# Qiyuan-Ge/PaintMind

Measured on AMD Instinct MI355X. Metric: 256x256 images/sec, 8-step MaskGIT decode (vit-s-vqgan), whole job, higher is better.
Workload: dtype bf16; 1 GPU; maskgit-uncond-12L-d512-T8; batch_per_gpu=64, topk=5, decode=every step (reference-equivalent work), parallelism=dp1 (independent images, no data-path collective), hip_graph=True, concurrent_micro_batches=2, dispatch_mode=AMD_DIRECT_DISPATCH=1 (default), rank_mode=False

## Files before the change

paintmind_amd/csrc/gemm.hip:

```cpp
#include <stdlib.h>

#include "gemm_common.h"

using namespace pmgemm;

int pm_gemm256_supported(const GemmParams& p, int dtype, int epi, int out_dtype);
int pm_gemm256_launch(const GemmParams& p, int epi, int out_dtype, hipStream_t s);
int pm_gemm2b_supported(const GemmParams& p, int dtype, int epi, int out_dtype);
int pm_gemm2b_launch(const GemmParams& p, int epi, int out_dtype, hipStream_t s);

namespace {

constexpr int BM = 128, BN = 128;
constexpr int TILE_BYTES = 128 * ROWB;
constexpr int STAGE_BYTES = 2 * TILE_BYTES;
constexpr int THREADS = 256;

template <typename T, int CH = 4>
__device__ __forceinline__ void stage_tile(const T* __restrict__ base, int ld, int row0, int rows_total,
                                           int k0, unsigned char* lds_tile, int wave, int lane) {
#pragma unroll
    for (int i = 0; i < CH; ++i) {
        const int chunk = wave * CH + i;
        const int r = chunk * 8 + (lane >> 3);
        const int slot = (lane & 7) ^ (r & 7);
        int gr = row0 + r;
        gr = gr < rows_total ? gr : rows_total - 1;
        const unsigned char* src =
            reinterpret_cast<const unsigned char*>(base + (size_t)gr * ld + k0) + slot * 16;
        glds16(src, lds_tile + chunk * 1024);
    }
}

template <typename T, int EPI, typename OutT, bool FOLD = false, int STAGES = 2, int WM = 2>
__global__ __launch_bounds__(WM * 128) void gemm_nt_kernel(const GemmParams p) {
    static_assert(STAGES == 2 || (STAGES == 4 && sizeof(T) == 2), "the four-stage K loop is the bf16 small-batch form");
    static_assert(WM == 2 || (WM == 4 && STAGES == 4), "eight waves only in the latency form");
    constexpr int MI = 8 / WM;
    constexpr int CH = 8 / WM;
    __shared__ __attribute__((aligned(1024))) unsigned char lds[STAGES * STAGE_BYTES];

    const int tid = threadIdx.x;
    const int lane = tid & 63;
    const int wave = __builtin_amdgcn_readfirstlane(tid >> 6);
    const int wm = wave >> 1, wn = wave & 1;
    const int l15 = lane & 15, g = lane >> 4;

    const int tiles_n = (p.N + BN - 1) / BN, tiles_m = (p.M + BM - 1) / BM;
    int tm, tn;
    tile_of_block(xcd_remap(blockIdx.x, gridDim.x), tiles_m, tiles_n, 8, tm, tn);
    const int m0 = tm * BM, n0 = tn * BN;

    const T* A = reinterpret_cast<const T*>(p.A);
    const T* W = reinterpret_cast<const T*>(p.W);
    constexpr int KSTEP = ROWB / (int)sizeof(T);
    const int nk = p.K / KSTEP;

    f32x4_t acc[MI][4];
#pragma unroll
    for (int i = 0; i < MI; ++i)
#pragma unroll
        for (int j = 0; j < 4; ++j) acc[i][j] = f32x4_t{0.f, 0.f, 0.f, 0.f};

    constexpr bool RPRE = (EPI == EPI_STD && sizeof(OutT) == 4);
    float4 rpre[RPRE ? MI * 4 : 1];
    if constexpr (RPRE) {
        if (p.residual) {
            const int ncol = n0 + wn * 64 + (lane & 15) * 4;
#pragma unroll
            for (int mi = 0; mi < MI; ++mi)
#pragma unroll
                for (int it = 0; it < 4; ++it) {
                    int mm = m0 + wm * (MI * 16) + mi * 16 + it * 4 + (lane >> 4);
                    mm = mm < p.M ? mm : p.M - 1;
                    const int nc = ncol < p.N ? ncol : 0;
                    rpre[mi * 4 + it] = *reinterpret_cast<const float4*>(p.residual + (size_t)(mm % p.res_rows) * p.ldr + nc);
                }
        }
    }

    stage_tile<T, CH>(A, p.lda, m0, p.M, 0, lds, wave, lane);
    stage_tile<T, CH>(W, p.ldw, n0, p.N, 0, lds + TILE_BYTES, wave, lane);

    [[maybe_unused]] float4 fcc[FOLD ? 4 : 1], fdd[FOLD ? 4 : 1];
    [[maybe_unused]] float2 fab[FOLD ? MI : 1];
    [[maybe_unused]] float2 fpa[FOLD && STAGES == 4 ? MI : 1][8], fpb[FOLD && STAGES == 4 ? MI : 1][8];
    if constexpr (FOLD) {
#pragma unroll
        for (int ni = 0; ni < 4; ++ni) {
            fcc[ni] = *reinterpret_cast<const float4*>(p.ln_c + n0 + wn * 64 + ni * 16 + g * 4);
// ... 114 lines not shown
        if (p.out_lo) { wave_epilogue<EPI, OutT, MI, 1, false, 2, NoHook, STAGES != 4>(p, acc, eraw, m0 + wm * (MI * 16), n0 + wn * 64, lane, rpre); return; }
    }
    wave_epilogue<EPI, OutT, MI, RPRE ? MI * 4 : 1, false, -1, NoHook, STAGES != 4>(p, acc, eraw, m0 + wm * (MI * 16), n0 + wn * 64, lane, rpre);
}

int tiles128(const GemmParams& p) { return ceil_div(p.M, BM) * ceil_div(p.N, BN); }


bool deep128(const GemmParams& p) {
    static const int deep_max = pm_dev_knob("PMHIP_GEMM128_DEEP_MAX_TILES", 256);
    return tiles128(p) <= deep_max && p.K >= 4 * 64;
}

template <typename T, int EPI, typename OutT, bool FOLD = false>
int launch(const GemmParams& p, bool deep, hipStream_t s) {
    const int tiles = tiles128(p);
    PmTimer tm(gemm_family(p, EPI), s);
    if constexpr (sizeof(T) == 2) {
        if (deep) {
            hipLaunchKernelGGL((gemm_nt_kernel<T, EPI, OutT, FOLD, 4, 4>), dim3(tiles), dim3(512), 0, s, p);
            PM_HIP(hipGetLastError());
            return PMHIP_OK;
        }
    }
    hipLaunchKernelGGL((gemm_nt_kernel<T, EPI, OutT, FOLD>), dim3(tiles), dim3(THREADS), 0, s, p);
    PM_HIP(hipGetLastError());
    return PMHIP_OK;
}

bool fold_small(const GemmParams& p) {
    static const int max_tiles = pm_dev_knob("PMHIP_FOLD128_MAX_TILES", 128);
    return (p.M / 256) * (p.N / 256) <= max_tiles;
}

bool use256(const GemmParams& p, int dtype, int epi, int out_dtype) {
    static const int g_use256 = pm_dev_knob("PMHIP_GEMM256", 1);
    return g_use256 && pm_gemm256_supported(p, dtype, epi, out_dtype);
}

bool use2b(const GemmParams& p, int dtype, int epi, int out_dtype) {
    static const int g_use2b = pm_dev_knob("PMHIP_GEMM2B", 1);
    if (!g_use2b || !pm_gemm2b_supported(p, dtype, epi, out_dtype)) return false;
    if (g_use2b >= 2) return true;
    return epi == EPI_STD && p.residual && !pm_gemm256_supported(p, dtype, epi, out_dtype);
}

int check_common(const GemmParams& p, int dtype) {
    PM_REQUIRE(dtype == PMHIP_F32 || dtype == PMHIP_BF16, "gemm: bad dtype %d", dtype);
    PM_REQUIRE(p.M > 0 && p.N > 0 && p.K > 0, "gemm: empty problem M=%d N=%d K=%d", p.M, p.N, p.K);
    PM_REQUIRE(p.K % 64 == 0, "gemm: K=%d must be a multiple of 64 (pad on the host)", p.K);
    PM_REQUIRE(p.lda % 8 == 0 && p.ldw % 8 == 0, "gemm: lda/ldw must be multiples of 8 elements");
    PM_REQUIRE(p.lda >= p.K, "gemm: lda=%d is smaller than K=%d (rows of A would overlap)", p.lda, p.K);
    PM_REQUIRE(p.ldw >= p.K, "gemm: ldw=%d is smaller than K=%d (rows of W would overlap)", p.ldw, p.K);
    PM_REQUIRE(p.A && p.W, "gemm: null operand");
    return PMHIP_OK;
}

int set_lnfold(GemmParams& p, const pmhip_lnfold* ln, int dtype) {
    PM_REQUIRE(ln->coef && ln->c && ln->d, "gemm_ln: null fold pointer");
    PM_REQUIRE(dtype == PMHIP_BF16, "gemm_ln: the LayerNorm fold exists in bf16 mode only");
    PM_REQUIRE(p.K % 128 == 0, "gemm_ln: K=%d must be a multiple of 128", p.K);
    p.ln_c = ln->c; p.ln_d = ln->d; p.ln_coef = ln->coef;
    PM_REQUIRE(pm_lnfold_shape_ok(p.M, p.N, p.K, p.lda, p.ldw),
               "gemm_ln: shape M=%d N=%d K=%d is not served by the 256x256 kernel (M, N multiples of 256)", p.M, p.N, p.K);
    PM_REQUIRE(!ln->parts || (ln->nparts > 0 && ln->nparts <= 16 && ln->nparts * 64 == p.K), "gemm_ln: nparts=%d does not describe K=%d columns",
               ln->nparts, p.K);
    return PMHIP_OK;
}

template <int EPI, bool FOLD>
int launch_bf16(const GemmParams& p, int out_dtype, bool deep, hipStream_t s) {
    if constexpr (EPI == EPI_STD)
        if (out_dtype == PMHIP_F32) return launch<bf16_t, EPI, float, FOLD>(p, deep, s);
    return launch<bf16_t, EPI, bf16_t, FOLD>(p, deep, s);
}

template <int EPI>
int dispatch(GemmParams& p, int dtype, int out_dtype, const pmhip_lnfold* ln, pmhip_stream stream) {
    hipStream_t s = (hipStream_t)stream;
    if (ln) {
        PM_TRY(set_lnfold(p, ln, dtype));
        const bool small = fold_small(p), deep = small && deep128(p);
        if (ln->parts) {
            if (deep) { p.ln_parts = ln->parts; p.ln_nparts = ln->nparts; p.ln_eps = ln->eps; p.ln_coef_out = const_cast<float*>(ln->coef); }
            else PM_TRY(pmhip_ln_coef_parts(ln->parts, ln->nparts, ln->eps, const_cast<float*>(ln->coef), p.M, stream));
        }
        if (small) return launch_bf16<EPI, true>(p, out_dtype, deep, s);
        return pm_gemm256_launch(p, EPI, out_dtype, s);
    }
    if (use2b(p, dtype, EPI, out_dtype)) return pm_gemm2b_launch(p, EPI, out_dtype, s);
    if (use256(p, dtype, EPI, out_dtype)) return pm_gemm256_launch(p, EPI, out_dtype, s);
    if (dtype == PMHIP_F32) return launch<float, EPI, float>(p, false, s);
    return launch_bf16<EPI, false>(p, out_dtype, deep128(p), s);
}

int gemm_impl(int dtype, const void* A, int lda, const void* W, int ldw, const float* bias,
                          const float* residual, int ldr, int res_rows, void* out, int ldo, int out_dtype,
                          int M, int N, int K, const pmhip_lnfold* ln, pmhip_stream stream, float* block_stats = nullptr) {
    GemmParams p{};
    p.A = A; p.W = W; p.bias = bias; p.residual = residual; p.out = out;
    p.block_stats = block_stats;
    PM_REQUIRE(!block_stats || (out_dtype == PMHIP_F32 && !residual && N % 64 == 0),
               "gemm_softmax_stats: block statistics need an f32 output without a residual and N=%d a multiple of 64", N);
    p.lda = lda; p.ldw = ldw; p.ldr = ldr; p.res_rows = res_rows > 0 ? res_rows : M; p.ldo = ldo;
    p.M = M; p.N = N; p.K = K;
    PM_TRY(check_common(p, dtype));
    PM_REQUIRE(out, "gemm: null out");
    PM_REQUIRE(N % 4 == 0 && ldo % 4 == 0, "gemm: N=%d and ldo=%d must be multiples of 4", N, ldo);
    PM_REQUIRE(ldo >= N, "gemm: ldo=%d is smaller than N=%d (rows of out would overlap)", ldo, N);
    PM_REQUIRE(!residual || ldr % 4 == 0, "gemm: ldr must be a multiple of 4");
    PM_REQUIRE(!residual || ldr >= N, "gemm: ldr=%d is smaller than N=%d (rows of the residual would overlap)", ldr, N);
    PM_REQUIRE(!residual || out_dtype == PMHIP_F32, "gemm: a residual needs an f32 output (the residual stream is f32)");
    PM_REQUIRE(out_dtype == PMHIP_F32 || out_dtype == dtype, "gemm: out dtype must be f32 or the compute dtype");
    PM_REQUIRE(out_dtype == PMHIP_F32 || ldo % 8 == 0, "gemm: bf16 output needs ldo to be a multiple of 8");
    return dispatch<EPI_STD>(p, dtype, out_dtype, ln, stream);
}

}

extern "C" int pmhip_gemm(int dtype, const void* A, int lda, const void* W, int ldw, const float* bias,
                          const float* residual, int ldr, int res_rows, void* out, int ldo, int out_dtype,
                          int M, int N, int K, pmhip_stream stream) {
    return gemm_impl(dtype, A, lda, W, ldw, bias, residual, ldr, res_rows, out, ldo, out_dtype, M, N, K, nullptr, stream);
}

static int gemm_hilo_impl(const void* A, int lda, const void* W, int ldw, const float* bias, const void* res_hi,
                          const void* res_lo, int ldr, int res_rows, void* out_hi, void* out_lo, int ldo, int M, int N, int K,
                          float* row_stats, pmhip_stream stream, const float* center_coef = nullptr, float center_extra = 0.f,
                          float* shift = nullptr, int shift_mode = 0) {
    GemmParams p{};
    p.center_coef = center_coef; p.center_extra = center_coef ? center_extra : 0.f; p.shift = shift; p.shift_mode = shift ? shift_mode : 0;
    PM_REQUIRE(shift_mode >= 0 && shift_mode <= 2, "gemm_hilo_center: shift_mode=%d", shift_mode);
    PM_REQUIRE(!(center_coef || shift_mode == 2) || res_rows <= 0 || res_rows >= M,
               "gemm_hilo_center: centring / shift accumulation needs the residual to be the stream itself (no row modulo)");
    p.A = A; p.W = W; p.bias = bias; p.residual = reinterpret_cast<const float*>(res_hi); p.out = out_hi;
    p.res_lo = reinterpret_cast<const bf16_t*>(res_lo); p.out_lo = reinterpret_cast<bf16_t*>(out_lo);
    p.lda = lda; p.ldw = ldw; p.ldr = ldr; p.res_rows = res_rows > 0 ? res_rows : M; p.ldo = ldo;
    p.M = M; p.N = N; p.K = K;
    p.row_stats = row_stats;
    PM_TRY(check_common(p, PMHIP_BF16));
    PM_REQUIRE(res_hi && res_lo && out_hi && out_lo, "gemm_hilo: null plane");
    PM_REQUIRE(N % 8 == 0 && ldo % 8 == 0 && ldr % 8 == 0, "gemm_hilo: N=%d, ldo=%d, ldr=%d must be multiples of 8", N, ldo, ldr);
    PM_REQUIRE(ldo >= N, "gemm_hilo: ldo=%d is smaller than N=%d (rows of the output planes would overlap)", ldo, N);
    PM_REQUIRE(ldr >= N, "gemm_hilo: ldr=%d is smaller than N=%d (rows of the residual planes would overlap)", ldr, N);
    PM_REQUIRE(!row_stats || N % 64 == 0, "gemm_hilo_stats: N=%d must be a multiple of 64", N);
    return dispatch<EPI_STD>(p, PMHIP_BF16, PMHIP_BF16, nullptr, stream);
}

extern "C" int pmhip_gemm_hilo(const void* A, int lda, const void* W, int ldw, const float* bias, const void* res_hi,
                               const void* res_lo, int ldr, int res_rows, void* out_hi, void* out_lo, int ldo, int M, int N, int K,
                               pmhip_stream stream) {
    return gemm_hilo_impl(A, lda, W, ldw, bias, res_hi, res_lo, ldr, res_rows, out_hi, out_lo, ldo, M, N, K, nullptr, stream);
}

extern "C" int pmhip_gemm_hilo_stats(const void* A, int lda, const void* W, int ldw, const float* bias, const void* res_hi,
                                     const void* res_lo, int ldr, int res_rows, void* out_hi, void* out_lo, int ldo, int M, int N,
                                     int K, float* row_stats, pmhip_stream stream) {
    PM_REQUIRE(row_stats, "gemm_hilo_stats: null statistics buffer");
    return gemm_hilo_impl(A, lda, W, ldw, bias, res_hi, res_lo, ldr, res_rows, out_hi, out_lo, ldo, M, N, K, row_stats, stream);
}

extern "C" int pmhip_gemm_hilo_center(const void* A, int lda, const void* W, int ldw, const float* bias, const void* res_hi,
                                      const void* res_lo, int ldr, int res_rows, void* out_hi, void* out_lo, int ldo, int M, int N,
                                      int K, float* row_stats, const float* center_coef, float center_extra, float* shift,
                                      int shift_mode, pmhip_stream stream) {
    return gemm_hilo_impl(A, lda, W, ldw, bias, res_hi, res_lo, ldr, res_rows, out_hi, out_lo, ldo, M, N, K, row_stats, stream, center_coef,
                          center_extra, shift, shift_mode);
}
// ... 78 lines not shown
```

paintmind_amd/csrc/gemm256.hip:

```cpp
#include <stdlib.h>

#include <mutex>

#include "gemm_common.h"

using namespace pmgemm;

namespace {

constexpr int BM = 256, BN = 256, THREADS = 512;
constexpr int OPER_BYTES = 256 * ROWB;
constexpr int BUF_BYTES = 2 * OPER_BYTES;
constexpr int KSTEP = ROWB / 2;

enum { PA0 = 0, PW0 = 1, PW1 = 2, PA1 = 3 };

__device__ __forceinline__ int piece_row(int piece, int c) {
    const int pr = c * 8;
    if (piece == PA0) return pr < 64 ? pr : 128 + (pr - 64);
    if (piece == PA1) return pr < 64 ? 64 + pr : 192 + (pr - 64);
    const int grp = pr >> 5, within = pr & 31;
    return grp * 64 + within + (piece == PW1 ? 32 : 0);
}

typedef __amdgpu_buffer_rsrc_t rsrc_t;
__device__ __forceinline__ rsrc_t tile_rsrc(const void* origin) {
    return __builtin_amdgcn_make_buffer_rsrc(const_cast<void*>(origin), 0, 0x7fffffff, 0x00020000);
}
__device__ __forceinline__ void issue_piece(int piece, rsrc_t Ar, rsrc_t Wr, unsigned aorg, unsigned worg, unsigned lda_b, unsigned ldw_b,
                                            unsigned laneoffA, unsigned laneoffW, int k0, unsigned char* buf, int wave, int i0 = 0, int i1 = 2) {
    const bool isA = (piece == PA0 || piece == PA1);
    const unsigned org = isA ? aorg : worg;
    const unsigned ld_b = isA ? lda_b : ldw_b;
    const unsigned laneoff = isA ? laneoffA : laneoffW;
    unsigned char* tile = buf + (isA ? 0 : OPER_BYTES);
#pragma unroll
    for (int i = i0; i < i1; ++i) {
        const int row0 = piece_row(piece, wave * 2 + i);
        const unsigned soff = org + (unsigned)row0 * ld_b + (unsigned)k0 * 2u;
        __builtin_amdgcn_raw_ptr_buffer_load_lds(isA ? Ar : Wr, (__attribute__((address_space(3))) void*)(tile + row0 * ROWB), 16, laneoff,
                                                 soff, 0, 0);
    }
}

struct LoopCtx {
    rsrc_t Ar, Wr;
    unsigned aorg, worg;
    unsigned aorg1, worg1;
    unsigned lda_b, ldw_b;
    unsigned laneoffA, laneoffW;
    unsigned fa0, fa1, fw0, fw1;
    unsigned lds_base;
    int nk, wave;
    int mw, nw, lane;
};


#define DSR(dst, addr, off) asm volatile("ds_read_b128 %0, %1 offset:%2" : "=v"(dst) : "v"(addr), "n"(off))
#define RD_A(half)                                                  \
    DSR(a[0][0], ba0, ((half) * 64 + 0) * ROWB);  DSR(a[0][1], ba1, ((half) * 64 + 0) * ROWB);  \
    DSR(a[1][0], ba0, ((half) * 64 + 16) * ROWB); DSR(a[1][1], ba1, ((half) * 64 + 16) * ROWB); \
    DSR(a[2][0], ba0, ((half) * 64 + 32) * ROWB); DSR(a[2][1], ba1, ((half) * 64 + 32) * ROWB); \
    DSR(a[3][0], ba0, ((half) * 64 + 48) * ROWB); DSR(a[3][1], ba1, ((half) * 64 + 48) * ROWB);
#define RD_W(half)                                                  \
    DSR(w[0][0], bw0, ((half) * 32 + 0) * ROWB);  DSR(w[0][1], bw1, ((half) * 32 + 0) * ROWB);  \
    DSR(w[1][0], bw0, ((half) * 32 + 16) * ROWB); DSR(w[1][1], bw1, ((half) * 32 + 16) * ROWB);
#define MMA(mhalf, nhalf)                                                                        \
    {                                                                                            \
        __builtin_amdgcn_s_setprio(1);                                                           \
        _Pragma("unroll") for (int kk = 0; kk < 2; ++kk) _Pragma("unroll") for (int f = 0; f < 4; ++f) \
            _Pragma("unroll") for (int h = 0; h < 2; ++h)                                        \
                Mma<bf16_t>::run(acc[(mhalf) * 4 + f][(nhalf) * 2 + h], w[h][kk], a[f][kk]);     \
        __builtin_amdgcn_s_setprio(0);                                                           \
    }
#define LGKM0 asm volatile("s_waitcnt lgkmcnt(0)" ::: "memory"); __builtin_amdgcn_sched_barrier(0)
#define BAR __builtin_amdgcn_s_barrier()
#define VMW(n) { __builtin_amdgcn_sched_barrier(0); asm volatile("s_waitcnt vmcnt(" #n ")" ::: "memory"); __builtin_amdgcn_sched_barrier(0); }

enum { KT_STEADY = 0, KT_FIRST = 1, KT_LAST = 2 };

template <bool LEAD, int KIND, bool FOLD>
__device__ __forceinline__ void k_tile(const GemmParams& p, const LoopCtx& c, unsigned char* lds, f32x4_t (&acc)[8][4], uint4 (&a)[4][2],
                                       uint4 (&w)[2][2], float* fscr, int kt, int pb) {
#ifdef PM_FOLD_DIRECT
    constexpr bool FOLD_DIRECT = true;
#else
    constexpr bool FOLD_DIRECT = false;
#endif
    constexpr int XL = (FOLD && !FOLD_DIRECT && KIND == KT_LAST) ? LN_COEF_LOADS : 0;
    constexpr bool FIRST = KIND == KT_FIRST;
    constexpr bool ONE_PER_PHASE = KIND != KT_LAST;
    const unsigned boff = (unsigned)((kt + pb) & 1) * BUF_BYTES;
    const unsigned ba0 = c.lds_base + boff + c.fa0, ba1 = c.lds_base + boff + c.fa1;
    const unsigned bw0 = c.lds_base + boff + c.fw0, bw1 = c.lds_base + boff + c.fw1;
    unsigned char* nxt = lds + ((kt + 1 + pb) & 1) * BUF_BYTES;
#define ISSUE(piece) issue_piece(piece, c.Ar, c.Wr, c.aorg, c.worg, c.lda_b, c.ldw_b, c.laneoffA, c.laneoffW, (kt + 1) * KSTEP, nxt, c.wave);
#define ISSUE_NEXT_TILE(piece) issue_piece(piece, c.Ar, c.Wr, c.aorg1, c.worg1, c.lda_b, c.ldw_b, c.laneoffA, c.laneoffW, 0, nxt, c.wave);
#define DMA(phase)                                                                                                   \
    if constexpr (ONE_PER_PHASE) {                                                                                   \
        if constexpr (phase == 1) { ISSUE(PA0) } else if constexpr (phase == 2) { ISSUE(PW0) }                       \
        else if constexpr (phase == 3) { ISSUE(PW1) } else { ISSUE(PA1) }                                            \
    } else {                                                                                                         \
        if constexpr (phase == 1 && FOLD) ln_coef_issue(p, c.mw, c.nw, c.lane, fscr);                                 \
        if constexpr (phase == 1) { ISSUE_NEXT_TILE(PA0) ISSUE_NEXT_TILE(PW0) }                                      \
        else if constexpr (phase == 2) { ISSUE_NEXT_TILE(PW1) ISSUE_NEXT_TILE(PA1) }                                 \
    }
#define WAIT(phase)                                                                                                  \
    if constexpr (KIND == KT_STEADY) VMW(4)                                                                          \
    else if constexpr (KIND == KT_FIRST) { if constexpr (phase == 4) VMW(4) }                                        \
    else if constexpr (XL == 0) {                                                                                    \
        if constexpr (phase == 1) VMW(6) else if constexpr (phase == 2) VMW(8) else if constexpr (phase == 4) VMW(0) \
    } else {                                                                                                         \
        if constexpr (phase == 1) VMW(9) else if constexpr (phase == 2) VMW(11) else if constexpr (phase == 4) VMW(0) \
    }
    constexpr bool LATE_DMA1 = KIND == KT_LAST;
    if constexpr (LEAD) { RD_A(0) RD_W(0) if constexpr (!LATE_DMA1) { DMA(1) } } else if constexpr (!FIRST) { LGKM0; MMA(1, 0) }
    BAR;
    if constexpr (LEAD) { LGKM0; MMA(0, 0) if constexpr (LATE_DMA1) { DMA(1) } } else { RD_A(0) RD_W(0) DMA(1) }
    WAIT(1)
    BAR;
    if constexpr (LEAD) { RD_W(1) DMA(2) } else { LGKM0; MMA(0, 0) }
    BAR;
    if constexpr (LEAD) { LGKM0; MMA(0, 1) } else { RD_W(1) DMA(2) }
    WAIT(2)
    BAR;
    if constexpr (LEAD) { RD_A(1) DMA(3) } else { LGKM0; MMA(0, 1) }
    BAR;
    if constexpr (LEAD) { LGKM0; MMA(1, 1) } else { RD_A(1) DMA(3) }
    WAIT(3)
    BAR;
    if constexpr (LEAD) { RD_W(0) DMA(4) } else { LGKM0; MMA(1, 1) }
    BAR;
    if constexpr (LEAD) { LGKM0; MMA(1, 0) } else { RD_W(0) DMA(4) }
    WAIT(4)
    BAR;
#undef ISSUE
#undef ISSUE_NEXT_TILE
#undef DMA
#undef WAIT
}

template <bool LEAD, bool FOLD>
__device__ __forceinline__ void k_loop(const GemmParams& p, const LoopCtx& c, unsigned char* lds, f32x4_t (&acc)[8][4], float* fscr, int pb) {
    uint4 a[4][2], w[2][2];
    k_tile<LEAD, KT_FIRST, FOLD>(p, c, lds, acc, a, w, fscr, 0, pb);
    for (int kt = 1; kt + 1 < c.nk; ++kt) k_tile<LEAD, KT_STEADY, FOLD>(p, c, lds, acc, a, w, fscr, kt, pb);
    k_tile<LEAD, KT_LAST, FOLD>(p, c, lds, acc, a, w, fscr, c.nk - 1, pb);
    if constexpr (!LEAD) { LGKM0; MMA(1, 0) }
}
#undef DSR
#undef RD_A
#undef RD_W
#undef MMA
#undef LGKM0
#undef BAR
#undef VMW


template <int EPI, typename OutT, bool FOLD = false>
__global__ __launch_bounds__(THREADS) void gemm256_kernel(const GemmParams p) {
    __shared__ __attribute__((aligned(1024))) unsigned char lds[2 * BUF_BYTES + (FOLD ? 8 * 2048 : 0)];

    const int tid = threadIdx.x;
    const int lane = tid & 63;
    const int wave = __builtin_amdgcn_readfirstlane(tid >> 6);
    const int wm = wave >> 2, wn = wave & 3;
    const int l15 = lane & 15, g = lane >> 4;

    const int ntiles = (p.M / BM) * (p.N / BN);
    const int tiles_m = p.M / BM, tiles_n = p.N / BN;
    LoopCtx c;
    c.lda_b = (unsigned)p.lda * 2u; c.ldw_b = (unsigned)p.ldw * 2u;
    const unsigned lswz = (unsigned)(((lane & 7) ^ ((lane >> 3) & 7)) << 4);
    c.laneoffA = (unsigned)(lane >> 3) * (unsigned)c.lda_b + lswz;
    c.laneoffW = (unsigned)(lane >> 3) * (unsigned)c.ldw_b + lswz;
    c.fa0 = (unsigned)((wm * 128 + l15) * ROWB) + ((unsigned)((0 + g) ^ (l15 & 7)) << 4);
    c.fa1 = (unsigned)((wm * 128 + l15) * ROWB) + ((unsigned)((4 + g) ^ (l15 & 7)) << 4);
    c.fw0 = (unsigned)(OPER_BYTES + (wn * 64 + l15) * ROWB) + ((unsigned)((0 + g) ^ (l15 & 7)) << 4);
    c.fw1 = (unsigned)(OPER_BYTES + (wn * 64 + l15) * ROWB) + ((unsigned)((4 + g) ^ (l15 & 7)) << 4);
    c.nk = p.K / KSTEP;
    c.wave = wave;
    c.lds_base = (unsigned)(size_t)(__attribute__((address_space(3))) unsigned char*)lds;

    auto origin = [&](int tile, int& m0, int& n0) {
        int tm, tn;
        tile_of_block(xcd_remap(tile, ntiles), tiles_m, tiles_n, p.chunk, tm, tn);
        m0 = tm * BM; n0 = tn * BN;
    };
    int tile = blockIdx.x, m0, n0;
    origin(tile, m0, n0);
    c.Ar = tile_rsrc(p.A);
    c.Wr = tile_rsrc(p.W);
    c.aorg = (unsigned)m0 * c.lda_b; c.worg = (unsigned)n0 * c.ldw_b;

    issue_piece(PA0, c.Ar, c.Wr, c.aorg, c.worg, c.lda_b, c.ldw_b, c.laneoffA, c.laneoffW, 0, lds, wave);
    issue_piece(PW0, c.Ar, c.Wr, c.aorg, c.worg, c.lda_b, c.ldw_b, c.laneoffA, c.laneoffW, 0, lds, wave);
    issue_piece(PW1, c.Ar, c.Wr, c.aorg, c.worg, c.lda_b, c.ldw_b, c.laneoffA, c.laneoffW, 0, lds, wave);
    issue_piece(PA1, c.Ar, c.Wr, c.aorg, c.worg, c.lda_b, c.ldw_b, c.laneoffA, c.laneoffW, 0, lds, wave);
    float* fscr = reinterpret_cast<float*>(lds + 2 * BUF_BYTES + (FOLD ? wave * 2048 : 0));
    c.lane = lane;
    asm volatile("s_waitcnt vmcnt(0)" ::: "memory");
    __builtin_amdgcn_s_barrier();

    int pb = 0;
    for (;;) {
        f32x4_t acc[8][4];
#pragma unroll
        for (int i = 0; i < 8; ++i)
#pragma unroll
            for (int j = 0; j < 4; ++j) acc[i][j] = f32x4_t{0.f, 0.f, 0.f, 0.f};

        const int next = tile + (int)gridDim.x;
        const bool has_next = next < ntiles;
        int m1 = m0, n1 = n0;
        if (has_next) origin(next, m1, n1);
        c.aorg1 = (unsigned)m1 * c.lda_b; c.worg1 = (unsigned)n1 * c.ldw_b;

        c.mw = m0 + wm * 128; c.nw = n0 + wn * 64;
        if (wm == 0) k_loop<true, FOLD>(p, c, lds, acc, fscr, pb); else k_loop<false, FOLD>(p, c, lds, acc, fscr, pb);

#if defined(PM_FOLD_NOAPPLY)
#elif defined(PM_FOLD_DIRECT)
        if constexpr (FOLD) ln_apply_direct<8>(p, c.mw, c.nw, acc, lane);
#else
        if constexpr (FOLD) ln_apply<8>(fscr, acc, lane);
#endif
        const float4 no_pre[1] = {};
        unsigned char* eraw = lds + ((pb + c.nk - 1) & 1) * BUF_BYTES + wave * EPI_WAVE_BYTES;
        const int mw = m0 + wm * 128, nw = n0 + wn * 64;
        if constexpr (EPI == EPI_STD && sizeof(OutT) == 4) {
            if (p.residual) wave_epilogue<EPI, OutT, 8, 1, true, 1>(p, acc, eraw, mw, nw, lane, no_pre);
            else wave_epilogue<EPI, OutT, 8, 1, true, 0>(p, acc, eraw, mw, nw, lane, no_pre);
        } else if constexpr (EPI == EPI_STD) {
            if (!FOLD && p.out_lo) wave_epilogue<EPI, OutT, 8, 1, true, 2>(p, acc, eraw, mw, nw, lane, no_pre);
            else wave_epilogue<EPI, OutT, 8, 1, true, 0>(p, acc, eraw, mw, nw, lane, no_pre);
        } else {
            wave_epilogue<EPI, OutT, 8, 1, true, 0>(p, acc, eraw, mw, nw, lane, no_pre);
        }
        if (!has_next) break;
        __builtin_amdgcn_s_barrier();
        tile = next; m0 = m1; n0 = n1;
        c.aorg = c.aorg1; c.worg = c.worg1;
        pb = (pb + c.nk) & 1;
    }
}

struct Knobs256 {
    int chunk = 6;
    int persist = 256;
    int res_kmin = 1024;
};
const Knobs256& knobs256() {
    static Knobs256 k;
    static std::once_flag once;
    std::call_once(once, [] {
        k.chunk = pm_dev_knob("PMHIP_CHUNK256", k.chunk);
        k.persist = pm_dev_knob("PMHIP_PERSIST256", k.persist);
        k.res_kmin = pm_dev_knob("PMHIP_G256_RES_KMIN", k.res_kmin);
    });
    return k;
}

template <int EPI, typename OutT>
int launch256(const GemmParams& p0, hipStream_t s) {
    GemmParams p = p0;
    p.chunk = knobs256().chunk;
    const int tiles = (p.M / BM) * (p.N / BN);
    const int persist = knobs256().persist;
    const int grid = (persist > 0 && tiles > persist) ? persist : tiles;
    if (p.ln_coef && p.out_lo) { pm_set_error("gemm256: a hi/lo residual producer cannot have a LayerNorm folded in"); return PMHIP_EINVAL; }
    PmTimer tm(gemm_family(p, EPI), s);
    if (p.ln_coef) hipLaunchKernelGGL((gemm256_kernel<EPI, OutT, true>), dim3(grid), dim3(THREADS), 0, s, p);
    else hipLaunchKernelGGL((gemm256_kernel<EPI, OutT, false>), dim3(grid), dim3(THREADS), 0, s, p);
    PM_HIP(hipGetLastError());
    return PMHIP_OK;
}

}

int pm_gemm256_supported(const GemmParams& p, int dtype, int epi, int out_dtype) {
    if (dtype != PMHIP_BF16) return 0;
    if (p.M % BM || p.N % BN || p.K % KSTEP || p.K < 2 * KSTEP) return 0;
    if ((unsigned long long)p.M * p.lda * 2 >= (1ull << 31) || (unsigned long long)p.N * p.ldw * 2 >= (1ull << 31)) return 0;
    if ((p.M / BM) * (p.N / BN) < 96) return 0;
    if (epi == EPI_STD && p.residual) {
        if (p.K < knobs256().res_kmin) return 0;
    }
    (void)out_dtype;
    return 1;
}

int pm_gemm256_launch(const GemmParams& p, int epi, int out_dtype, hipStream_t s) {
    if (epi == EPI_SWIGLU) return launch256<EPI_SWIGLU, bf16_t>(p, s);
    if (epi == EPI_HEADS) return launch256<EPI_HEADS, bf16_t>(p, s);
    if (out_dtype == PMHIP_F32) return launch256<EPI_STD, float>(p, s);
    return launch256<EPI_STD, bf16_t>(p, s);
}
```

paintmind_amd/csrc/gemm_common.h:

```cpp
#pragma once
#include "common.h"

namespace pmgemm {

constexpr int ROWB = 128;
constexpr int ESTRIDE = 68;
constexpr int EPI_WAVE_BYTES = 8192;

enum { EPI_STD = 0, EPI_SWIGLU = 1, EPI_HEADS = 2 };

struct GemmParams {
    const void* A; const void* W;
    const float* bias; const float* residual;
    void* out;
    int lda, ldw, ldr, res_rows, ldo;
    int M, N, K;
    int heads, tokens, tokens_pad, inner;
    int kinds[3];
    void* outs[3];
    float q_scale;
    int fast_math;
    int chunk;
    const bf16_t* res_lo; bf16_t* out_lo;
    float* row_stats;
    const float* center_coef; float center_extra; float* shift; int shift_mode;
    const float* ln_coef;
    const float* ln_c; const float* ln_d;
    const float* ln_parts; int ln_nparts; float ln_eps; float* ln_coef_out;
    float* block_stats;
};

inline int gemm_family(const GemmParams& p, int epi, bool two_wg = false) {
    if (epi == EPI_HEADS) return FAM_GEMM_HEADS;
    if (epi == EPI_SWIGLU) return FAM_GEMM_SWIGLU;
    if (p.residual || p.out_lo) return two_wg ? FAM_GEMM_RESID2B : FAM_GEMM_RESID;
    return FAM_GEMM;
}

__device__ __forceinline__ int xcd_remap(int bid, int nblocks) {
    const int q = nblocks >> 3, r = nblocks & 7;
    const int xcd = bid & 7, local = bid >> 3;
    const int base = (xcd < r) ? xcd * (q + 1) : r * (q + 1) + (xcd - r) * q;
    return base + local;
}

__device__ __forceinline__ void tile_of_block(int vb, int tiles_m, int tiles_n, int max_chunk, int& tm, int& tn) {
    const int nchunks = (tiles_n + max_chunk - 1) / max_chunk;
    const int cw = (tiles_n + nchunks - 1) / nchunks;
    const int chunk = vb / (tiles_m * cw);
    const int cw_here = min(cw, tiles_n - chunk * cw);
    const int rem = vb - chunk * tiles_m * cw;
    tm = rem / cw_here;
    tn = chunk * cw + rem % cw_here;
}

__device__ __forceinline__ uint4 read_frag(const unsigned char* lds_tile, int row, int slot) {
    return *reinterpret_cast<const uint4*>(lds_tile + row * ROWB + ((slot ^ (row & 7)) << 4));
}

__device__ __forceinline__ float silu_mul_fast(float x1, float x2) {
    return x1 * __builtin_amdgcn_rcpf(1.0f + __builtin_amdgcn_exp2f(x1 * -1.4426950408889634f)) * x2;
}
__device__ __forceinline__ float silu_mul(float x1, float x2, int fast) {
    if (fast) return silu_mul_fast(x1, x2);
    return (x1 / (1.0f + expf(-x1))) * x2;
}

constexpr int LN_COEF_LOADS = 3;
__device__ __forceinline__ void ln_coef_issue(const GemmParams& p, int mwave, int nw, int lane, float* scratch) {
    typedef __attribute__((address_space(3))) void lds_void;
    typedef const __attribute__((address_space(1))) void gbl_void;
    __builtin_amdgcn_global_load_lds((gbl_void*)(p.ln_coef + (size_t)mwave * 2 + lane * 4), (lds_void*)scratch, 16, 0, 0);
    __builtin_amdgcn_global_load_lds((gbl_void*)(p.ln_c + nw + lane), (lds_void*)(scratch + 256), 4, 0, 0);
    __builtin_amdgcn_global_load_lds((gbl_void*)(p.ln_d + nw + lane), (lds_void*)(scratch + 320), 4, 0, 0);
}

typedef float pk2_t __attribute__((ext_vector_type(2)));
__device__ __forceinline__ pk2_t pk_splat(float v) {
    float lo, hi;
    asm("v_mov_b32 %0, %1" : "=v"(lo) : "v"(v));
    asm("v_mov_b32 %0, %1" : "=v"(hi) : "v"(v));
    return pk2_t{lo, hi};
}
__device__ __forceinline__ pk2_t pk_fma_plain(pk2_t a, pk2_t b, pk2_t c) {
    pk2_t d;
    asm("v_pk_fma_f32 %0, %1, %2, %3" : "=v"(d) : "v"(a), "v"(b), "v"(c));
    return d;
}
__device__ __forceinline__ void ln_apply4(f32x4_t& acc, pk2_t xx, pk2_t yy, const float4& c, const float4& d) {
    const pk2_t t0 = pk_fma_plain(pk2_t{c.x, c.y}, yy, pk2_t{d.x, d.y}), t1 = pk_fma_plain(pk2_t{c.z, c.w}, yy, pk2_t{d.z, d.w});
    const pk2_t o0 = pk_fma_plain(xx, pk2_t{acc[0], acc[1]}, t0), o1 = pk_fma_plain(xx, pk2_t{acc[2], acc[3]}, t1);
    acc[0] = o0[0]; acc[1] = o0[1]; acc[2] = o1[0]; acc[3] = o1[1];
}

template <int MI>
__device__ __forceinline__ void ln_apply(const float* scratch, f32x4_t (&acc)[MI][4], int lane) {
    const int g = lane >> 4, l15 = lane & 15;
    float4 cc[4], dd[4];
#pragma unroll
    for (int ni = 0; ni < 4; ++ni) {
        cc[ni] = *reinterpret_cast<const float4*>(scratch + 256 + ni * 16 + g * 4);
        dd[ni] = *reinterpret_cast<const float4*>(scratch + 320 + ni * 16 + g * 4);
    }
#pragma unroll
    for (int mi = 0; mi < MI; ++mi) {
        const float2 ab = *reinterpret_cast<const float2*>(scratch + (mi * 16 + l15) * 2);
        const pk2_t xx = pk_splat(ab.x), yy = pk_splat(ab.y);
#pragma unroll
        for (int ni = 0; ni < 4; ++ni) ln_apply4(acc[mi][ni], xx, yy, cc[ni], dd[ni]);
    }
}

template <int MI>
__device__ __forceinline__ void ln_apply_direct(const GemmParams& p, int mwave, int nw, f32x4_t (&acc)[MI][4], int lane) {
    const int g = lane >> 4, l15 = lane & 15;
    float4 cc[4], dd[4];
#pragma unroll
    for (int ni = 0; ni < 4; ++ni) {
        cc[ni] = *reinterpret_cast<const float4*>(p.ln_c + nw + ni * 16 + g * 4);
        dd[ni] = *reinterpret_cast<const float4*>(p.ln_d + nw + ni * 16 + g * 4);
    }
    float2 ab[MI];
#pragma unroll
    for (int mi = 0; mi < MI; ++mi) ab[mi] = *reinterpret_cast<const float2*>(p.ln_coef + (size_t)(mwave + mi * 16 + l15) * 2);
#pragma unroll
    for (int mi = 0; mi < MI; ++mi) {
        const pk2_t xx = pk_splat(ab[mi].x), yy = pk_splat(ab[mi].y);
#pragma unroll
        for (int ni = 0; ni < 4; ++ni) ln_apply4(acc[mi][ni], xx, yy, cc[ni], dd[ni]);
    }
}


typedef unsigned nt_v4u __attribute__((ext_vector_type(4)));
typedef unsigned nt_v2u __attribute__((ext_vector_type(2)));
__device__ __forceinline__ void nt_store16(void* p, uint4 v) {
    __builtin_nontemporal_store(nt_v4u{v.x, v.y, v.z, v.w}, reinterpret_cast<nt_v4u*>(p));
}
__device__ __forceinline__ void nt_store_row(float* p, const float (&v)[4]) { nt_store16(p, make_uint4(__float_as_uint(v[0]), __float_as_uint(v[1]), __float_as_uint(v[2]), __float_as_uint(v[3]))); }
__device__ __forceinline__ void nt_store_row(bf16_t* p, const float (&v)[8]) {
    nt_store16(p, make_uint4(pack_bf16x2(v[0], v[1]), pack_bf16x2(v[2], v[3]), pack_bf16x2(v[4], v[5]), pack_bf16x2(v[6], v[7])));
}
struct NoHook { __device__ __forceinline__ void operator()() const {} };
template <bool NT> __device__ __forceinline__ void st16(void* p, uint4 v) {
    if constexpr (NT) nt_store16(p, v);
    else *reinterpret_cast<uint4*>(p) = v;
}
template <bool NT> __device__ __forceinline__ void st_row(float* p, const float (&v)[4]) { st16<NT>(p, make_uint4(__float_as_uint(v[0]), __float_as_uint(v[1]), __float_as_uint(v[2]), __float_as_uint(v[3]))); }
template <bool NT> __device__ __forceinline__ void st_row(bf16_t* p, const float (&v)[8]) {
    st16<NT>(p, make_uint4(pack_bf16x2(v[0], v[1]), pack_bf16x2(v[2], v[3]), pack_bf16x2(v[4], v[5]), pack_bf16x2(v[6], v[7])));
}

template <int EPI, typename OutT, int MI, int NPRE, bool FULL = false, int RES = -1, typename Hook = NoHook, bool NT = true>
__device__ __forceinline__ void wave_epilogue(const GemmParams& p, f32x4_t (&acc)[MI][4], unsigned char* eraw, int mwave,
                                              int nw, int lane, const float4 (&rpre)[NPRE], Hook hook = Hook()) {
    constexpr int CPL = 16 / (int)sizeof(OutT);
    constexpr int LPR = 64 / CPL, RPI = 64 / LPR, ITERS = 16 / RPI;
    const int l15 = lane & 15, g = lane >> 4;
    const int ccol = (lane % LPR) * CPL, ncol = nw + ccol;
    float* ebuf = reinterpret_cast<float*>(eraw);
    if (!FULL && nw >= p.N) return;

    if constexpr (EPI == EPI_HEADS) {
        static_assert(MI % 4 == 0 || MI == 2, "the head-split epilogue transposes V in blocks of 64 (or 32) tokens");
        if (p.kinds[nw / p.inner] == PMHIP_PART_V) {
            hook();
            constexpr int TB = MI >= 4 ? 64 : MI * 16;
            constexpr int MIB = TB / 16;
            constexpr int LPRV = TB / 8, RPIV = 64 / LPRV, ITV = 64 / RPIV;
            const int h = (nw % p.inner) >> 6;
            OutT* dst = reinterpret_cast<OutT*>(p.outs[nw / p.inner]);
#pragma unroll
            for (int blk = 0; blk < MI / MIB; ++blk) {
                const int mblk = mwave + blk * TB;
                const int b0 = mblk / p.tokens, t0 = mblk % p.tokens;
                const bool whole = (FULL || mblk + TB - 1 < p.M) && (t0 + TB - 1 < p.tokens) && (t0 % 8 == 0);
                if (whole && sizeof(OutT) == 2) {
                    OutT* vbuf = reinterpret_cast<OutT*>(eraw);
#pragma unroll
                    for (int mi = 0; mi < MIB; ++mi)
#pragma unroll
                        for (int ni = 0; ni < 4; ++ni)
#pragma unroll
                            for (int r = 0; r < 4; ++r)
                                vbuf[(ni * 16 + g * 4 + r) * TB + mi * 16 + l15] = from_f32<OutT>(acc[blk * MIB + mi][ni][r]);
                    __builtin_amdgcn_wave_barrier();
                    asm volatile("s_waitcnt lgkmcnt(0)" ::: "memory");
                    OutT* vptr = dst + (((size_t)b0 * p.heads + h) * 64 + (lane / LPRV)) * p.tokens_pad + t0 + (lane % LPRV) * 8;
                    const unsigned char* lptr = eraw + (lane / LPRV) * (TB * 2) + (lane % LPRV) * 16;
// ... 364 lines not shown
```

Before: 547.3 images/s.

## Combine LayerNorm partial statistics inside the 256-tile GEMM instead of a separate kernel

For the large-tile GEMM with a folded LayerNorm, the per-row partial statistics are now loaded into LDS during the last K tile and combined in-kernel. The kernel also writes the resulting coefficients out from the n0==0 tiles, replacing the separate pmhip_ln_coef_parts launch. This removes one kernel launch and one global round trip per folded GEMM. In exchange it uses more LDS, adds combine work and extra vmcnt waits in the last K tile, and adds a template variant.

```diff
diff --git a/paintmind_amd/csrc/gemm.hip b/paintmind_amd/csrc/gemm.hip
--- a/paintmind_amd/csrc/gemm.hip
+++ b/paintmind_amd/csrc/gemm.hip
@@ -6,6 +6,7 @@
 
 int pm_gemm256_supported(const GemmParams& p, int dtype, int epi, int out_dtype);
 int pm_gemm256_launch(const GemmParams& p, int epi, int out_dtype, hipStream_t s);
+int pm_gemm256_combines_parts(int nparts);
 int pm_gemm2b_supported(const GemmParams& p, int dtype, int epi, int out_dtype);
 int pm_gemm2b_launch(const GemmParams& p, int epi, int out_dtype, hipStream_t s);
 
@@ -286,8 +287,9 @@
         PM_TRY(set_lnfold(p, ln, dtype));
         const bool small = fold_small(p), deep = small && deep128(p);
         if (ln->parts) {
-            if (deep) { p.ln_parts = ln->parts; p.ln_nparts = ln->nparts; p.ln_eps = ln->eps; p.ln_coef_out = const_cast<float*>(ln->coef); }
-            else PM_TRY(pmhip_ln_coef_parts(ln->parts, ln->nparts, ln->eps, const_cast<float*>(ln->coef), p.M, stream));
+            if (deep || (!small && pm_gemm256_combines_parts(ln->nparts))) {
+                p.ln_parts = ln->parts; p.ln_nparts = ln->nparts; p.ln_eps = ln->eps; p.ln_coef_out = const_cast<float*>(ln->coef);
+            } else PM_TRY(pmhip_ln_coef_parts(ln->parts, ln->nparts, ln->eps, const_cast<float*>(ln->coef), p.M, stream));
         }
         if (small) return launch_bf16<EPI, true>(p, out_dtype, deep, s);
         return pm_gemm256_launch(p, EPI, out_dtype, s);
diff --git a/paintmind_amd/csrc/gemm256.hip b/paintmind_amd/csrc/gemm256.hip
--- a/paintmind_amd/csrc/gemm256.hip
+++ b/paintmind_amd/csrc/gemm256.hip
@@ -5,6 +5,8 @@
 #include "gemm_common.h"
 
 using namespace pmgemm;
+
+int pm_gemm256_combines_parts(int nparts);
 
 namespace {
 
@@ -76,10 +78,11 @@
 #define LGKM0 asm volatile("s_waitcnt lgkmcnt(0)" ::: "memory"); __builtin_amdgcn_sched_barrier(0)
 #define BAR __builtin_amdgcn_s_barrier()
 #define VMW(n) { __builtin_amdgcn_sched_barrier(0); asm volatile("s_waitcnt vmcnt(" #n ")" ::: "memory"); __builtin_amdgcn_sched_barrier(0); }
+#define VMWC(n) { __builtin_amdgcn_sched_barrier(0); asm volatile("s_waitcnt vmcnt(%0)" :: "n"(n) : "memory"); __builtin_amdgcn_sched_barrier(0); }
 
 enum { KT_STEADY = 0, KT_FIRST = 1, KT_LAST = 2 };
 
-template <bool LEAD, int KIND, bool FOLD>
+template <bool LEAD, int KIND, bool FOLD, bool PARTS>
 __device__ __forceinline__ void k_tile(const GemmParams& p, const LoopCtx& c, unsigned char* lds, f32x4_t (&acc)[8][4], uint4 (&a)[4][2],
                                        uint4 (&w)[2][2], float* fscr, int kt, int pb) {
 #ifdef PM_FOLD_DIRECT
@@ -87,7 +90,7 @@
 #else
     constexpr bool FOLD_DIRECT = false;
 #endif
-    constexpr int XL = (FOLD && !FOLD_DIRECT && KIND == KT_LAST) ? LN_COEF_LOADS : 0;
+    constexpr int XL = (FOLD && !FOLD_DIRECT && KIND == KT_LAST) ? (PARTS ? LN_PARTS_LOADS : LN_COEF_LOADS) : 0;
     constexpr bool FIRST = KIND == KT_FIRST;
     constexpr bool ONE_PER_PHASE = KIND != KT_LAST;
     const unsigned boff = (unsigned)((kt + pb) & 1) * BUF_BYTES;
@@ -101,7 +104,8 @@
         if constexpr (phase == 1) { ISSUE(PA0) } else if constexpr (phase == 2) { ISSUE(PW0) }                       \
         else if constexpr (phase == 3) { ISSUE(PW1) } else { ISSUE(PA1) }                                            \
     } else {                                                                                                         \
-        if constexpr (phase == 1 && FOLD) ln_coef_issue(p, c.mw, c.nw, c.lane, fscr);                                 \
+        if constexpr (phase == 1 && FOLD && PARTS) ln_parts_issue(p, c.mw, c.wave & 3, c.nw, c.lane, fscr);           \
+        else if constexpr (phase == 1 && FOLD) ln_coef_issue(p, c.mw, c.nw, c.lane, fscr);                            \
         if constexpr (phase == 1) { ISSUE_NEXT_TILE(PA0) ISSUE_NEXT_TILE(PW0) }                                      \
         else if constexpr (phase == 2) { ISSUE_NEXT_TILE(PW1) ISSUE_NEXT_TILE(PA1) }                                 \
     }
@@ -111,8 +115,12 @@
     else if constexpr (XL == 0) {                                                                                    \
         if constexpr (phase == 1) VMW(6) else if constexpr (phase == 2) VMW(8) else if constexpr (phase == 4) VMW(0) \
     } else {                                                                                                         \
-        if constexpr (phase == 1) VMW(9) else if constexpr (phase == 2) VMW(11) else if constexpr (phase == 4) VMW(0) \
-    }
+        if constexpr (phase == 1) VMWC(6 + XL) else if constexpr (phase == 2) VMWC(8 + XL)                           \
+        else if constexpr (phase == 3 && PARTS) VMWC(8) else if constexpr (phase == 4) VMW(0)                        \
+    }
+    constexpr bool COMBINE = XL > 0 && PARTS;
+#define COMBINE_PARTS                                                                                                \
+    if constexpr (COMBINE) ln_parts_combine(p, fscr, reinterpret_cast<float*>(lds + 2 * BUF_BYTES), (c.wave >> 2) * 128 + (c.wave & 3) * 32, c.lane);
     constexpr bool LATE_DMA1 = KIND == KT_LAST;
     if constexpr (LEAD) { RD_A(0) RD_W(0) if constexpr (!LATE_DMA1) { DMA(1) } } else if constexpr (!FIRST) { LGKM0; MMA(1, 0) }
     BAR;
@@ -129,23 +137,24 @@
     if constexpr (LEAD) { LGKM0; MMA(1, 1) } else { RD_A(1) DMA(3) }
     WAIT(3)
     BAR;
-    if constexpr (LEAD) { RD_W(0) DMA(4) } else { LGKM0; MMA(1, 1) }
-    BAR;
-    if constexpr (LEAD) { LGKM0; MMA(1, 0) } else { RD_W(0) DMA(4) }
+    if constexpr (LEAD) { RD_W(0) DMA(4) COMBINE_PARTS } else { LGKM0; MMA(1, 1) }
+    BAR;
+    if constexpr (LEAD) { LGKM0; MMA(1, 0) } else { RD_W(0) DMA(4) COMBINE_PARTS if constexpr (COMBINE) { LGKM0; } }
     WAIT(4)
     BAR;
 #undef ISSUE
 #undef ISSUE_NEXT_TILE
 #undef DMA
 #undef WAIT
-}
-
-template <bool LEAD, bool FOLD>
+#undef COMBINE_PARTS
+}
+
+template <bool LEAD, bool FOLD, bool PARTS>
 __device__ __forceinline__ void k_loop(const GemmParams& p, const LoopCtx& c, unsigned char* lds, f32x4_t (&acc)[8][4], float* fscr, int pb) {
     uint4 a[4][2], w[2][2];
-    k_tile<LEAD, KT_FIRST, FOLD>(p, c, lds, acc, a, w, fscr, 0, pb);
-    for (int kt = 1; kt + 1 < c.nk; ++kt) k_tile<LEAD, KT_STEADY, FOLD>(p, c, lds, acc, a, w, fscr, kt, pb);
-    k_tile<LEAD, KT_LAST, FOLD>(p, c, lds, acc, a, w, fscr, c.nk - 1, pb);
+    k_tile<LEAD, KT_FIRST, FOLD, PARTS>(p, c, lds, acc, a, w, fscr, 0, pb);
+    for (int kt = 1; kt + 1 < c.nk; ++kt) k_tile<LEAD, KT_STEADY, FOLD, PARTS>(p, c, lds, acc, a, w, fscr, kt, pb);
+    k_tile<LEAD, KT_LAST, FOLD, PARTS>(p, c, lds, acc, a, w, fscr, c.nk - 1, pb);
     if constexpr (!LEAD) { LGKM0; MMA(1, 0) }
 }
 #undef DSR
@@ -155,11 +164,16 @@
 #undef LGKM0
 #undef BAR
 #undef VMW
-
-
-template <int EPI, typename OutT, bool FOLD = false>
+#undef VMWC
+
+
+constexpr int FOLD_LDS = 8 * 2048;
+constexpr int FOLD_PARTS_LDS = LN_SHARED_BYTES + 8 * LN_PARTS_WAVE_BYTES;
+
+template <int EPI, typename OutT, bool FOLD = false, bool PARTS = false>
 __global__ __launch_bounds__(THREADS) void gemm256_kernel(const GemmParams p) {
-    __shared__ __attribute__((aligned(1024))) unsigned char lds[2 * BUF_BYTES + (FOLD ? 8 * 2048 : 0)];
+    static_assert(FOLD || !PARTS, "partial statistics belong to a folded LayerNorm");
+    __shared__ __attribute__((aligned(1024))) unsigned char lds[2 * BUF_BYTES + (FOLD ? (PARTS ? FOLD_PARTS_LDS : FOLD_LDS) : 0)];
 
     const int tid = threadIdx.x;
     const int lane = tid & 63;
@@ -197,7 +211,8 @@
     issue_piece(PW0, c.Ar, c.Wr, c.aorg, c.worg, c.lda_b, c.ldw_b, c.laneoffA, c.laneoffW, 0, lds, wave);
     issue_piece(PW1, c.Ar, c.Wr, c.aorg, c.worg, c.lda_b, c.ldw_b, c.laneoffA, c.laneoffW, 0, lds, wave);
     issue_piece(PA1, c.Ar, c.Wr, c.aorg, c.worg, c.lda_b, c.ldw_b, c.laneoffA, c.laneoffW, 0, lds, wave);
-    float* fscr = reinterpret_cast<float*>(lds + 2 * BUF_BYTES + (FOLD ? wave * 2048 : 0));
+    float* fscr = reinterpret_cast<float*>(lds + 2 * BUF_BYTES + (FOLD ? (PARTS ? LN_SHARED_BYTES + wave * LN_PARTS_WAVE_BYTES : wave * 2048) : 0));
+    [[maybe_unused]] float* fshared = reinterpret_cast<float*>(lds + 2 * BUF_BYTES);
     c.lane = lane;
     asm volatile("s_waitcnt vmcnt(0)" ::: "memory");
     __builtin_amdgcn_s_barrier();
@@ -217,13 +232,17 @@
         c.aorg1 = (unsigned)m1 * c.lda_b; c.worg1 = (unsigned)n1 * c.ldw_b;
 
         c.mw = m0 + wm * 128; c.nw = n0 + wn * 64;
-        if (wm == 0) k_loop<true, FOLD>(p, c, lds, acc, fscr, pb); else k_loop<false, FOLD>(p, c, lds, acc, fscr, pb);
+        if (wm == 0) k_loop<true, FOLD, PARTS>(p, c, lds, acc, fscr, pb); else k_loop<false, FOLD, PARTS>(p, c, lds, acc, fscr, pb);
 
 #if defined(PM_FOLD_NOAPPLY)
 #elif defined(PM_FOLD_DIRECT)
         if constexpr (FOLD) ln_apply_direct<8>(p, c.mw, c.nw, acc, lane);
 #else
-        if constexpr (FOLD) ln_apply<8>(fscr, acc, lane);
+        if constexpr (FOLD && PARTS) {
+            ln_apply<8>(fshared + wm * 256, fscr + 512, acc, lane);
+        } else if constexpr (FOLD) {
+            ln_apply<8>(fscr, fscr + 256, acc, lane);
+        }
 #endif
         const float4 no_pre[1] = {};
         unsigned char* eraw = lds + ((pb + c.nk - 1) & 1) * BUF_BYTES + wave * EPI_WAVE_BYTES;
@@ -236,6 +255,11 @@
             else wave_epilogue<EPI, OutT, 8, 1, true, 0>(p, acc, eraw, mw, nw, lane, no_pre);
         } else {
             wave_epilogue<EPI, OutT, 8, 1, true, 0>(p, acc, eraw, mw, nw, lane, no_pre);
+        }
+        if constexpr (FOLD && PARTS) {
+            const int trow = wm * 128 + wn * 32;
+            if (n0 == 0 && lane < 32)
+                reinterpret_cast<float2*>(p.ln_coef_out)[(size_t)(m0 + trow + lane)] = *reinterpret_cast<const float2*>(fshared + (trow + lane) * 2);
         }
         if (!has_next) break;
         __builtin_amdgcn_s_barrier();
@@ -270,7 +294,10 @@
     const int grid = (persist > 0 && tiles > persist) ? persist : tiles;
     if (p.ln_coef && p.out_lo) { pm_set_error("gemm256: a hi/lo residual producer cannot have a LayerNorm folded in"); return PMHIP_EINVAL; }
     PmTimer tm(gemm_family(p, EPI), s);
-    if (p.ln_coef) hipLaunchKernelGGL((gemm256_kernel<EPI, OutT, true>), dim3(grid), dim3(THREADS), 0, s, p);
+    if (p.ln_parts) {
+        if (!pm_gemm256_combines_parts(p.ln_nparts) || !p.ln_coef_out) { pm_set_error("gemm256: partial statistics this kernel does not combine"); return PMHIP_EINVAL; }
+        hipLaunchKernelGGL((gemm256_kernel<EPI, OutT, true, true>), dim3(grid), dim3(THREADS), 0, s, p);
+    } else if (p.ln_coef) hipLaunchKernelGGL((gemm256_kernel<EPI, OutT, true>), dim3(grid), dim3(THREADS), 0, s, p);
     else hipLaunchKernelGGL((gemm256_kernel<EPI, OutT, false>), dim3(grid), dim3(THREADS), 0, s, p);
     PM_HIP(hipGetLastError());
     return PMHIP_OK;
@@ -290,6 +317,14 @@
     return 1;
 }
 
+int pm_gemm256_combines_parts(int nparts) {
+#if defined(PM_FOLD_NOAPPLY) || defined(PM_FOLD_DIRECT)
+    return 0;
+#else
+    return nparts == LN_PARTS;
+#endif
+}
+
 int pm_gemm256_launch(const GemmParams& p, int epi, int out_dtype, hipStream_t s) {
     if (epi == EPI_SWIGLU) return launch256<EPI_SWIGLU, bf16_t>(p, s);
     if (epi == EPI_HEADS) return launch256<EPI_HEADS, bf16_t>(p, s);
diff --git a/paintmind_amd/csrc/gemm_common.h b/paintmind_amd/csrc/gemm_common.h
--- a/paintmind_amd/csrc/gemm_common.h
+++ b/paintmind_amd/csrc/gemm_common.h
@@ -75,6 +75,33 @@
     __builtin_amdgcn_global_load_lds((gbl_void*)(p.ln_d + nw + lane), (lds_void*)(scratch + 320), 4, 0, 0);
 }
 
+constexpr int LN_PARTS = 8;
+constexpr int LN_PARTS_LOADS = 4;
+constexpr int LN_PARTS_WAVE_BYTES = 32 * LN_PARTS * 8 + 512;
+constexpr int LN_SHARED_BYTES = 256 * 8;
+__device__ __forceinline__ void ln_parts_issue(const GemmParams& p, int mwave, int wn, int nw, int lane, float* scratch) {
+    typedef __attribute__((address_space(3))) void lds_void;
+    typedef const __attribute__((address_space(1))) void gbl_void;
+    const float* src = p.ln_parts + (size_t)(mwave + wn * 32) * (LN_PARTS * 2) + lane * 4;
+    __builtin_amdgcn_global_load_lds((gbl_void*)src, (lds_void*)scratch, 16, 0, 0);
+    __builtin_amdgcn_global_load_lds((gbl_void*)(src + 256), (lds_void*)(scratch + 256), 16, 0, 0);
+    __builtin_amdgcn_global_load_lds((gbl_void*)(p.ln_c + nw + lane), (lds_void*)(scratch + 512), 4, 0, 0);
+    __builtin_amdgcn_global_load_lds((gbl_void*)(p.ln_d + nw + lane), (lds_void*)(scratch + 576), 4, 0, 0);
+}
+__device__ __forceinline__ void ln_parts_combine(const GemmParams& p, const float* scratch, float* shared, int trow, int lane) {
+    const int r = lane & 31;
+    float2 pa[8], pb[8];
+#pragma unroll
+    for (int j = 0; j < LN_PARTS / 2; ++j) {
+        const float4 v = *reinterpret_cast<const float4*>(scratch + r * (LN_PARTS * 2) + j * 4);
+        pa[2 * j] = make_float2(v.x, v.y); pa[2 * j + 1] = make_float2(v.z, v.w);
+    }
+#pragma unroll
+    for (int j = 0; j < 8; ++j) pb[j] = make_float2(0.f, 0.f);
+    const float2 ab = ln_coef_row(pa, pb, LN_PARTS, p.ln_eps);
+    if (lane < 32) *reinterpret_cast<float2*>(shared + (trow + r) * 2) = ab;
+}
+
 typedef float pk2_t __attribute__((ext_vector_type(2)));
 __device__ __forceinline__ pk2_t pk_splat(float v) {
     float lo, hi;
@@ -94,17 +121,17 @@
 }
 
 template <int MI>
-__device__ __forceinline__ void ln_apply(const float* scratch, f32x4_t (&acc)[MI][4], int lane) {
+__device__ __forceinline__ void ln_apply(const float* rows, const float* cd, f32x4_t (&acc)[MI][4], int lane) {
     const int g = lane >> 4, l15 = lane & 15;
     float4 cc[4], dd[4];
 #pragma unroll
     for (int ni = 0; ni < 4; ++ni) {
-        cc[ni] = *reinterpret_cast<const float4*>(scratch + 256 + ni * 16 + g * 4);
-        dd[ni] = *reinterpret_cast<const float4*>(scratch + 320 + ni * 16 + g * 4);
+        cc[ni] = *reinterpret_cast<const float4*>(cd + ni * 16 + g * 4);
+        dd[ni] = *reinterpret_cast<const float4*>(cd + 64 + ni * 16 + g * 4);
     }
 #pragma unroll
     for (int mi = 0; mi < MI; ++mi) {
-        const float2 ab = *reinterpret_cast<const float2*>(scratch + (mi * 16 + l15) * 2);
+        const float2 ab = *reinterpret_cast<const float2*>(rows + (mi * 16 + l15) * 2);
         const pk2_t xx = pk_splat(ab.x), yy = pk_splat(ab.y);
 #pragma unroll
         for (int ni = 0; ni < 4; ++ni) ln_apply4(acc[mi][ni], xx, yy, cc[ni], dd[ni]);
```

After: 541.4 images/s. -1.1%, worse.
